# balisujohn/tortoise.cpp

Hardware: AMD Instinct MI355X
Metric: audio-seconds/sec end-to-end (AR+diffusion+vocoder), 16 cands x 80 steps (higher is better)
Workload: dtype f16 MFMA inputs / f32 accumulate (diffusion, vocoder convs); f32 weights, f16 KV (AR)

## Files before the change

tortoise.cpp_amd/csrc/diffusion.hip:

```cpp
#include "common.h"
#include "gemm_f16.h"
#include <algorithm>
#include <chrono>
#include <cmath>

namespace tts {

static constexpr int C = 1024, NHEAD = 16, XTC = 128 ;
static constexpr int LAT_MAX_ROWS = 2048;
static constexpr int HOIST_MAX_ROWS = 16384;

__device__ __forceinline__ float silu_dev(float x, int lut) {
  if (lut == 1) {
    float xr = __half2float(__float2half_rn(x));
    return __half2float(__float2half_rn(xr / (1.0f + expf(-xr))));
  }
  if (lut == 2) return x / (1.0f + expf(-x));
  return x * __builtin_amdgcn_rcpf(1.0f + __builtin_amdgcn_exp2f(x * -1.44269504088896f));
}

__global__ __launch_bounds__(256) void gn_stats_kernel(const float *__restrict__ x, const int *__restrict__ seq_start,
                                                       const int *__restrict__ seq_len, float eps, float2 *__restrict__ stats) {
  __shared__ float sh[8];
  const int grp = blockIdx.x, s = blockIdx.y, T = seq_len[s];
// ... 1213 lines not shown
    if (g.mode == GEMM_OUT_QKV) fam = "diff_gemm_qkv";
    else if (gemm_is_conv3(g) && g.N == C && g.kseg == C) fam = g.resid ? "diff_gemm_k3r" : "diff_gemm_k3";
    else if (g.nseg == 1 && g.N == C && g.kseg == C && g.mode == GEMM_OUT_F32) fam = g.resid ? "diff_gemm_k1r" : "diff_gemm_k1";
    else if (g.custom_w && g.N == C && g.kseg == C && g.mode == GEMM_OUT_F32_SCALED && g.resid) fam = "diff_gemm_k1r";
    else fam = "diff_gemm_misc";
  }
  ProfScope ps(ctx, fam, 2.0 * mv * (n_valid ? n_valid : g.N) * (k_valid ? k_valid : g.nseg * g.kseg));
  TTS_HIP(ctx, launch_gemm_f16(g, ctx->stream));
  if (ctx->fp16_check) {
    if (gemm_mode_qkv(g.mode)) {
      CHECK(fp16_check(ctx, g.outH, (size_t)g.M * g.ldh));
      CHECK(fp16_check(ctx, g.outVt, (size_t)(g.N / 3) * g.ldvt));
    } else if (g.mode == GEMM_OUT_F16) CHECK(fp16_check(ctx, g.outH, (size_t)g.M * g.ldh));
  }
  return TTS_OK;
}

static int gemm_wreg_class(const tts_ctx *ctx, int bit) { return (ctx->gemm_wreg & bit) ? 1 : 0; }
static const __half *gemm_wreg_image(const tts_ctx *ctx, int bit, const Layout &lay, int N, const __half *w, const __half *wf) {
  return gemm_wreg_class(ctx, bit) && gemm_auto_th(lay.rows, N) == 8 ? wf : w;
}

static GemmArgs gemm_base(const Layout &lay, const __half *A, int lda, int nseg, int kseg, const __half *W, int N,
                          const float *bias) {
  GemmArgs g{};
  for (int i = 0; i < 3; i++) { g.A[i] = A; g.row_off[i] = 0; }
  if (nseg == 3) { g.row_off[0] = -1; g.row_off[1] = 0; g.row_off[2] = 1; }
  g.nseg = nseg; g.kseg = kseg; g.lda = lda; g.W = W; g.M = lay.rows; g.N = N; g.bias = bias;
  g.row_seq = lay.d_row_seq.as<int>();
  return g;
}

static int gn_stats(tts_ctx *ctx, const Layout &lay, Work &wk, const float *x) {
  ProfScope ps(ctx, "diff_gn_stats");
  gn_stats_kernel<<<dim3(32, lay.ns), 256, 0, ctx->stream>>>(x, lay.d_start.as<int>(), lay.d_len.as<int>(), ctx->gn_eps,
                                                             wk.stats.as<float2>());
  TTS_HIP(ctx, hipGetLastError());
  return TTS_OK;
}
template <int NT, int NJ, class LOAD, class TOUCH>
__device__ __forceinline__ void gn_reg_body(LOAD load, TOUCH touch, int s, int c, int T, int r0, const int *__restrict__ seq_start, int rows_total, int ns, float eps,
                                            const float *__restrict__ g, const float *__restrict__ b, const float *__restrict__ ss, int do_silu, int lut,
                                            __half *__restrict__ y, const int *__restrict__ seq_step, int ss_step_stride) {
  constexpr int NW = NT / 64, SWEEP = NT / 8;
  __shared__ float sh[2][NW];
  const int t0 = threadIdx.x >> 3;
  float4 v[NJ];
#pragma unroll
  for (int j = 0; j < NJ; j++) {
    const int t = t0 + j * SWEEP;
    v[j] = load(min(t, T - 1));
  }
  touch();
  const float4 gg = *(const float4 *)(g + c), bb = *(const float4 *)(b + c);
  float sc4[4] = {1.f, 1.f, 1.f, 1.f}, sh4[4] = {0.f, 0.f, 0.f, 0.f};
  if (ss) {
    if (seq_step) ss += (size_t)seq_step[s] * ss_step_stride;
#pragma unroll
    for (int i = 0; i < 4; i++) { sc4[i] = ss[c + i] + 1.0f; sh4[i] = ss[C + c + i]; }
  }
  float sum = 0.f;
#pragma unroll
  for (int j = 0; j < NJ; j++)
    if (t0 + j * SWEEP < T) sum += (v[j].x + v[j].y) + (v[j].z + v[j].w);
#pragma unroll
  for (int o = 32; o > 0; o >>= 1) sum += __shfl_xor(sum, o);
  if ((threadIdx.x & 63) == 0) sh[0][threadIdx.x >> 6] = sum;
  __syncthreads();
  float tot = 0.f;
#pragma unroll
  for (int w = 0; w < NW; w++) tot += sh[0][w];
  const float n = (float)T * 32.f, mean = tot / n;
  float sq = 0.f;
#pragma unroll
  for (int j = 0; j < NJ; j++) {
    v[j].x -= mean; v[j].y -= mean; v[j].z -= mean; v[j].w -= mean;
    if (t0 + j * SWEEP < T) sq += (v[j].x * v[j].x + v[j].y * v[j].y) + (v[j].z * v[j].z + v[j].w * v[j].w);
  }
#pragma unroll
  for (int o = 32; o > 0; o >>= 1) sq += __shfl_xor(sq, o);
  if ((threadIdx.x & 63) == 0) sh[1][threadIdx.x >> 6] = sq;
  __syncthreads();
  float tsq = 0.f;
#pragma unroll
  for (int w = 0; w < NW; w++) tsq += sh[1][w];
  const float rstd = 1.0f / sqrtf(tsq / n + eps);
  const float ge[4] = {gg.x, gg.y, gg.z, gg.w}, be[4] = {bb.x, bb.y, bb.z, bb.w};
  auto apply = [&](auto mode) {
    constexpr int MODE = decltype(mode)::value;
#pragma unroll
    for (int j = 0; j < NJ; j++) {
      const int t = min(t0 + j * SWEEP, T - 1);
      float e[4] = {v[j].x, v[j].y, v[j].z, v[j].w};
#pragma unroll
      for (int i = 0; i < 4; i++) {
        float u = e[i] * rstd;
        u = u * ge[i];
        u = u + be[i];
        u = u * sc4[i];
        u = u + sh4[i];
        if (MODE) u = silu_dev(u, MODE - 1);
        e[i] = u;
      }
      const __half2 p0 = __floats2half2_rn(e[0], e[1]), p1 = __floats2half2_rn(e[2], e[3]);
      uint2 o;
      o.x = *(const unsigned *)&p0;
      o.y = *(const unsigned *)&p1;
      *(uint2 *)(y + (size_t)(r0 + t) * C + c) = o;
    }
  };
  if (!do_silu) apply(std::integral_constant<int, 0>{});
  else if (lut == 0) apply(std::integral_constant<int, 1>{});
  else if (lut == 1) apply(std::integral_constant<int, 2>{});
  else apply(std::integral_constant<int, 3>{});
  const int gend = (s + 1 < ns) ? seq_start[s + 1] : rows_total;
  for (int r = r0 + T + t0; r < gend; r += SWEEP) *(uint2 *)(y + (size_t)r * C + c) = make_uint2(0u, 0u);
  if (s == 0)
    for (int r = t0; r < r0; r += SWEEP) *(uint2 *)(y + (size_t)r * C + c) = make_uint2(0u, 0u);
}
template <int NT, int NJ>
__global__ __launch_bounds__(NT) void gn_reg_kernel(const float *__restrict__ x, const int *__restrict__ seq_start,
                                                    const int *__restrict__ seq_len, int rows_total, int ns, float eps,
                                                    const float *__restrict__ g, const float *__restrict__ b,
                                                    const float *__restrict__ ss, int do_silu, int lut, __half *__restrict__ y,
                                                    const char *__restrict__ pf0, int pf0_lines, const char *__restrict__ pf1, int pf1_lines,
                                                    const int *__restrict__ seq_step, int ss_step_stride) {
  constexpr int NW = NT / 64;
  __shared__ unsigned pf_sink[NW][64];
  const int bid = blockIdx.y * 32 + blockIdx.x, nbk = ns * 32, item = (bid & 7) * (nbk >> 3) + (bid >> 3);
  const int s = item >> 5, grp = item & 31;
  const int T = seq_len[s], r0 = seq_start[s];
  const int q = threadIdx.x & 7, c = grp * 32 + q * 4;
  const float *base = x + (size_t)r0 * C + c;
  auto touch = [&]() {
    const int gi = (blockIdx.y * 32 + blockIdx.x) * NT + threadIdx.x, tt = 32 * ns * NT;
    unsigned *sink = &pf_sink[__builtin_amdgcn_readfirstlane(threadIdx.x >> 6)][0];
    for (int l = gi; l < pf0_lines; l += tt) __builtin_amdgcn_global_load_lds((gptr_t)(pf0 + (size_t)l * 128), (lptr_t)sink, 4, 0, 0);
    for (int l = gi; l < pf1_lines; l += tt) __builtin_amdgcn_global_load_lds((gptr_t)(pf1 + (size_t)l * 128), (lptr_t)sink, 4, 0, 0);
  };
  gn_reg_body<NT, NJ>([&](int t) { return *(const float4 *)(base + (size_t)t * C); }, touch, s, c, T, r0, seq_start, rows_total, ns, eps, g, b, ss, do_silu, lut, y, seq_step,
                      ss_step_stride);
  if (pf0_lines | pf1_lines) asm volatile("s_waitcnt vmcnt(0)" ::: "memory");
}
struct GnPanelTail {
  __device__ __forceinline__ void operator()(const GemmGnPanelArgs &a, int s, int T, int r0, int c0, const char *panel) const {
    const int q = threadIdx.x & 7;
    gn_reg_body<512, 14>([&](int t) { return *(const float4 *)(panel + gnp_panel_f4(t, q)); }, []() {}, s, c0 + q * 4, T, r0, a.seq_start, a.rows_total, a.ns, a.eps, a.gn_g,
                         a.gn_b, a.ss, a.do_silu, a.lut, a.y, a.seq_step, a.ss_step_stride);
  }
};

static inline hipError_t launch_gemm_gn_panel(const GemmGnPanelArgs &a, hipStream_t s) {
  static bool raised = false;
  if (!raised) { (void)hipFuncSetAttribute((const void *)gemm_f16_gn_panel_kernel<GnPanelTail>, hipFuncAttributeMaxDynamicSharedMemorySize, GEMM_GN_PANEL_LDS); raised = true; }
  gemm_f16_gn_panel_kernel<GnPanelTail><<<gemm_gn_panel_grid(a.ns, a.N), 512, GEMM_GN_PANEL_LDS, s>>>(a, GnPanelTail{});
  return hipGetLastError();
}

static int gn_fused(tts_ctx *ctx, const Layout &lay, const float *x, const float *g, const float *b, const float *ss, int do_silu,
                    __half *y, const void *wa = nullptr, size_t wa_bytes = 0, const void *wb = nullptr, size_t wb_bytes = 0) {
  ProfScope ps(ctx, "diff_gn_fused");
  if (lay.rows > 4096) { wa_bytes = 0; wb_bytes = 0; }
  const int silu_mode = ctx->ggml_lut ? 1 : ctx->attn_f32 ? 2 : 0;
  auto launch = [&](const int *d_start, int s0, int ns, int row0, int rows, int tmax) {
    const float *xp = x + (size_t)row0 * C;
    __half *yp = y + (size_t)row0 * C;
    const int *d_len = lay.d_len.as<int>() + s0, *step = lay.seq_step_ptr() ? lay.seq_step_ptr() + s0 : nullptr;
#define GN_ARGS xp, d_start, d_len, rows, ns, ctx->gn_eps, g, b, ss, do_silu, silu_mode, yp, \
                (const char *)wa, (int)(wa_bytes >> 7), (const char *)wb, (int)(wb_bytes >> 7), step, lay.ss_step_stride
    if (tmax <= 14 * 64) gn_reg_kernel<512, 14><<<dim3(32, ns), 512, 0, ctx->stream>>>(GN_ARGS);
    else if (tmax <= 18 * 128) gn_reg_kernel<1024, 18><<<dim3(32, ns), 1024, 0, ctx->stream>>>(GN_ARGS);
    else gn_fused_kernel<0><<<dim3(32, ns), 256, 0, ctx->stream>>>(xp, d_start, d_len, rows, ns, ctx->gn_eps, g, b, ss,
                                                                  do_silu, silu_mode, yp, step, lay.ss_step_stride);
#undef GN_ARGS
  };
  if (lay.gn_parts.empty()) launch(lay.d_start.as<int>(), 0, lay.ns, 0, lay.rows, lay.max_len());
  else for (const Layout::GnPart &p : lay.gn_parts) launch(lay.d_start_rel.as<int>() + p.s0, p.s0, p.ns, p.row0, p.rows, p.tmax);
  TTS_HIP(ctx, hipGetLastError());
  return TTS_OK;
}

__global__ __launch_bounds__(256) void gn_apply_kernel(const float *__restrict__ x, const int *__restrict__ chunk_seq, const int *__restrict__ seq_start,
                                                       const int *__restrict__ seq_len, const long long *__restrict__ st, int stripe_ll, float eps, const float *__restrict__ g,
                                                       const float *__restrict__ b, const float *__restrict__ ss, int do_silu, int lut, __half *__restrict__ y,
                                                       const char *__restrict__ pf0, int pf0_lines, const char *__restrict__ pf1, int pf1_lines,
                                                       const int *__restrict__ seq_step, int ss_step_stride) {
  __shared__ float2 mr[32];
  __shared__ unsigned pf_sink[4][64];
  const int r0 = blockIdx.x * 4, s = chunk_seq[blockIdx.x >> 1], c = threadIdx.x * 4;
  float4 v[4];
#pragma unroll
  for (int r = 0; r < 4; r++) v[r] = *(const float4 *)(x + (size_t)(r0 + r) * C + c);
  {
    const int gi = blockIdx.x * 256 + threadIdx.x, tt = gridDim.x * 256;
    unsigned *sink = &pf_sink[__builtin_amdgcn_readfirstlane(threadIdx.x >> 6)][0];
    for (int l = gi; l < pf0_lines; l += tt) __builtin_amdgcn_global_load_lds((gptr_t)(pf0 + (size_t)l * 128), (lptr_t)sink, 4, 0, 0);
    for (int l = gi; l < pf1_lines; l += tt) __builtin_amdgcn_global_load_lds((gptr_t)(pf1 + (size_t)l * 128), (lptr_t)sink, 4, 0, 0);
  }
  int nvalid = 0;
  if (s >= 0) {
    nvalid = min(max(seq_start[s] + seq_len[s] - r0, 0), 4);
    if (threadIdx.x < 32) {
      long long a[4] = {0, 0, 0, 0};
      longlong2 u[FX_STRIPES][2];
#pragma unroll
      for (int k = 0; k < FX_STRIPES; k++) {
        const long long *sp = st + (size_t)k * stripe_ll + (size_t)(s * 32 + threadIdx.x) * 4;
        u[k][0] = *(const longlong2 *)sp; u[k][1] = *(const longlong2 *)(sp + 2);
      }
#pragma unroll
      for (int k = 0; k < FX_STRIPES; k++) { a[0] += u[k][0].x; a[1] += u[k][0].y; a[2] += u[k][1].x; a[3] += u[k][1].y; }
      const double n = (double)seq_len[s] * 32.0;
      const double mean = fx_value(a[0], a[1]) / n;
      const double var = fmax(fx_value(a[2], a[3]) / n - mean * mean, 0.0);
      mr[threadIdx.x] = make_float2((float)mean, (float)(1.0 / sqrt(var + (double)eps)));
    }
  }
  __syncthreads();
  const float2 m = mr[c >> 5];
  const float4 gg = *(const float4 *)(g + c), bb = *(const float4 *)(b + c);
  float sc4[4] = {1.f, 1.f, 1.f, 1.f}, sh4[4] = {0.f, 0.f, 0.f, 0.f};
  if (ss) {
    if (seq_step && s >= 0) ss += (size_t)seq_step[s] * ss_step_stride;
#pragma unroll
    for (int i = 0; i < 4; i++) { sc4[i] = ss[c + i] + 1.0f; sh4[i] = ss[C + c + i]; }
  }
  const float ge[4] = {gg.x, gg.y, gg.z, gg.w}, be[4] = {bb.x, bb.y, bb.z, bb.w};
  auto apply = [&](auto mode) {
    constexpr int MODE = decltype(mode)::value;
#pragma unroll
    for (int r = 0; r < 4; r++) {
      float e[4] = {v[r].x, v[r].y, v[r].z, v[r].w};
#pragma unroll
      for (int i = 0; i < 4; i++) {
        float u = (e[i] - m.x) * m.y;
        u = u * ge[i];
        u = u + be[i];
        u = u * sc4[i];
        u = u + sh4[i];
        if (MODE) u = silu_dev(u, MODE - 1);
        e[i] = r < nvalid ? u : 0.f;
      }
      const __half2 p0 = __floats2half2_rn(e[0], e[1]), p1 = __floats2half2_rn(e[2], e[3]);
      uint2 o;
      o.x = *(const unsigned *)&p0;
      o.y = *(const unsigned *)&p1;
      *(uint2 *)(y + (size_t)(r0 + r) * C + c) = o;
    }
  };
  if (!do_silu) apply(std::integral_constant<int, 0>{});
  else if (lut == 0) apply(std::integral_constant<int, 1>{});
  else if (lut == 1) apply(std::integral_constant<int, 2>{});
  else apply(std::integral_constant<int, 3>{});
  if (pf0_lines | pf1_lines) asm volatile("s_waitcnt vmcnt(0)" ::: "memory");
}

static int gn(tts_ctx *ctx, const DiffState *st, const Layout &lay, const float *x, const long long *st_x, const float *g, const float *b, const float *ss, int do_silu,
              __half *y, const void *wa = nullptr, size_t wa_bytes = 0, const void *wb = nullptr, size_t wb_bytes = 0) {
  if (!st_x) {
    CHECK(gn_fused(ctx, lay, x, g, b, ss, do_silu, y, wa, wa_bytes, wb, wb_bytes));
    return fp16_check(ctx, y, (size_t)lay.rows * C);
  }
  {
    ProfScope ps(ctx, "diff_gn_apply");
    const int silu_mode = ctx->ggml_lut ? 1 : ctx->attn_f32 ? 2 : 0;
    gn_apply_kernel<<<lay.rows / 4, 256, 0, ctx->stream>>>(x, lay.d_chunk_seq.as<int>(), lay.d_start.as<int>(), lay.d_len.as<int>(), st_x, (int)st->gn_stripe_ll, ctx->gn_eps, g, b,
                                                            ss, do_silu, silu_mode, y, (const char *)wa, (int)(wa_bytes >> 7), (const char *)wb, (int)(wb_bytes >> 7),
                                                            lay.seq_step_ptr(), lay.ss_step_stride);
    TTS_HIP(ctx, hipGetLastError());
  }
  return fp16_check(ctx, y, (size_t)lay.rows * C);
}

static int res_in_layers(tts_ctx *ctx, const DiffState *st, const Layout &lay, Work &wk, const float *x, const ResDev &w, float *H,
                         const long long *st_x = nullptr, long long *st_h_out = nullptr) {
  CHECK(gn(ctx, st, lay, x, st_x, w.in_g, w.in_b, nullptr, 1, wk.A16(), gemm_wreg_image(ctx, 1, lay, C, w.in_w, w.in_wf), (size_t)C * C * 2));
  DBG_SUM("res.in gn", wk.A16(), (size_t)lay.rows * C * 2);
  GemmArgs g = gemm_base(lay, wk.A16(), C, 1, C, w.in_w, C, w.in_bias);
  g.mode = st_h_out ? GEMM_OUT_F32_STATS : GEMM_OUT_F32; g.outF = H; g.ldo = C; g.resid = nullptr;
  g.Wf = w.in_wf; g.wreg = gemm_wreg_class(ctx, 1);
  g.st_out = st_h_out; g.st_stripe_ll = (int)st->gn_stripe_ll; g.chunk_seq = lay.d_chunk_seq.as<int>();
  CHECK(gemm(ctx, "diff_gemm", g, lay));
  DBG_SUM("res.in conv", H, (size_t)lay.rows * C * 4);
  return TTS_OK;
}

static int attention_block(tts_ctx *ctx, DiffState *st, const Layout &lay, Work &wk, float *X, const AttnDev &w, bool force_ref = false) {
  const bool f32 = ctx->attn_f32 != 0 || force_ref;
  const bool pw16 = !f32 && ctx->attn_proj_f16;
  const bool lat = st->lat && wk.st_x != nullptr;
  CHECK(gn(ctx, st, lay, X, lat ? wk.st_x : nullptr, w.norm_g, w.norm_b, nullptr, 0, wk.A16(), gemm_wreg_image(ctx, 2, lay, 3 * C, w.qkv_w, w.qkv_wf), (size_t)3 * C * C * 2, pw16 ? w.proj_w : w.proj_w_split,
           (size_t)C * C * (pw16 ? 2 : 4)));
  long long *st_out = lat ? st->new_stats_slot() : nullptr;
  wk.st_x = st_out;
  DBG_SUM("attn gn", wk.A16(), (size_t)lay.rows * C * 2);
  GemmArgs g = gemm_base(lay, wk.A16(), C, 1, C, w.qkv_w, 3 * C, w.qkv_b);
  g.mode = f32 ? GEMM_OUT_QKV_SPLIT : GEMM_OUT_QKV;
  g.Wf = w.qkv_wf; g.wreg = gemm_wreg_class(ctx, 2);
  g.outH = wk.qk16.as<__half>(); g.ldh = 2048; g.outVt = wk.vt16.as<__half>(); g.ldvt = wk.rows + 128;
  g.outH2 = wk.qk16_lo.as<__half>(); g.outVt2 = wk.vt16_lo.as<__half>();
  CHECK(gemm(ctx, "diff_gemm", g, lay));
  if (f32 && (ctx->attn_f32_drop & 1)) TTS_HIP(ctx, hipMemsetAsync(wk.qk16_lo.p, 0, (size_t)(wk.rows + 128) * 2048 * 2, ctx->stream));
  if (f32 && (ctx->attn_f32_drop & 2)) TTS_HIP(ctx, hipMemsetAsync(wk.vt16_lo.p, 0, (size_t)C * (wk.rows + 128) * 2, ctx->stream));
  DBG_SUM("attn qk", wk.qk16.p, (size_t)lay.rows * 2048 * 2);
  DBG_SUM("attn vt", wk.vt16.p, (size_t)C * (wk.rows + 128) * 2);
  {
    double aw = 0;
    for (int l : lay.len) aw += 4.0 * l * (double)l * 64 * NHEAD;
// ... 920 lines not shown
```

tortoise.cpp_amd/csrc/gemm_f16.h:

```cpp
#pragma once
#include <hip/hip_fp16.h>
#include <hip/hip_runtime.h>
#include <algorithm>
#include <cmath>
#include <cstdlib>
#include <type_traits>

namespace tts {

typedef _Float16 half8 __attribute__((ext_vector_type(8)));
typedef float floatx4 __attribute__((ext_vector_type(4)));

enum { GEMM_OUT_F32 = 0, GEMM_OUT_F16 = 1, GEMM_OUT_QKV = 2, GEMM_OUT_QKV_SPLIT = 3, GEMM_OUT_F32_SCALED = 4, GEMM_OUT_F32_STATS = 5, GEMM_OUT_F32_SCALED_STATS = 6 };
constexpr bool gemm_mode_qkv(int mode) { return mode == GEMM_OUT_QKV || mode == GEMM_OUT_QKV_SPLIT; }
constexpr bool gemm_mode_f32(int mode) { return mode == GEMM_OUT_F32 || mode == GEMM_OUT_F32_SCALED || mode == GEMM_OUT_F32_STATS || mode == GEMM_OUT_F32_SCALED_STATS; }
constexpr bool gemm_mode_scaled(int mode) { return mode == GEMM_OUT_F32_SCALED || mode == GEMM_OUT_F32_SCALED_STATS; }
constexpr bool gemm_mode_stats(int mode) { return mode == GEMM_OUT_F32_STATS || mode == GEMM_OUT_F32_SCALED_STATS; }

struct GemmArgs {
  const __half *A[3];
  int row_off[3];
  int nseg, kseg;
  int lda;
  const __half *W;
// ... 493 lines not shown
      return;
    }
  }
  const int col0 = c0 + fq * 4;
  float4 b4[2];
  int sq[MI];
#pragma unroll
  for (int j = 0; j < 2; j++) b4[j] = *(const float4 *)(bp + col0 + j * 16);
#pragma unroll
  for (int i = 0; i < MI; i++) sq[i] = sp[m0 + min(i, nblk - 1) * 16 + fr];
#pragma unroll
  for (int j = 0; j < 2; j++) b4[j] = hb ? b4[j] : make_float4(0.f, 0.f, 0.f, 0.f);
#pragma unroll
  for (int i = 0; i < MI; i++) sq[i] = hs ? sq[i] : 0;
  auto finish = [&](int i, int j) {
    float4 v = make_float4(acc[i][j][0] + b4[j].x, acc[i][j][1] + b4[j].y, acc[i][j][2] + b4[j].z, acc[i][j][3] + b4[j].w);
    if (sq[i] < 0) v = make_float4(0.f, 0.f, 0.f, 0.f);
    return v;
  };
  if (MODE == GEMM_OUT_F32) {
#pragma unroll
    for (int i = 0; i < MI; i++) {
      if (i < nblk) {
        float *op = g.outF + (size_t)(m0 + i * 16 + fr) * g.ldo + col0;
#pragma unroll
        for (int j = 0; j < 2; j++) *(float4 *)(op + j * 16) = finish(i, j);
      }
    }
  } else {
    const int h = c0 / 192, w0 = c0 - h * 192;
#pragma unroll
    for (int i = 0; i < MI; i++) {
      if (i < nblk) {
        __half *op = g.outH + (size_t)(m0 + i * 16 + fr) * g.ldh + h * 128 + w0 + fq * 4;
#pragma unroll
        for (int j = 0; j < 2; j++) {
          const float4 v = finish(i, j);
          *(uint2 *)(op + j * 16) = pack_half4(v.x, v.y, v.z, v.w);
          if (MODE == GEMM_OUT_QKV_SPLIT)
            *(uint2 *)(g.outH2 + (op - g.outH) + j * 16) = pack_half4(split_lo(v.x), split_lo(v.y), split_lo(v.z), split_lo(v.w));
        }
      }
    }
  }
}

template <int MODE, int MI, int D, bool NAT>
__device__ __forceinline__ void gemm_wreg_body(const GemmArgs &g, int m0, int n0, int nblk, int lane, int wave) {
  extern __shared__ __attribute__((aligned(16))) char smem_dyn[];
  char *smem = smem_dyn;
  constexpr int S = D + 1;
  constexpr int NPA = MI / 2;
  constexpr int PER = NPA + 4;
  static_assert(D == 1 || D == 2, "prefetch distance");
  const int T = g.kseg >> 6, KS = g.kseg >> 5;
  const int fr = lane & 15, fq = lane >> 4;
  unsigned aoff[NPA];
#pragma unroll
  for (int i = 0; i < NPA; i++) aoff[i] = (unsigned)(gemm_dma_off(wave + 4 * i, lane, 0, nblk * 16 - 1, g.lda) * 2);
  const char *aseg = (const char *)(g.A[0] + (ptrdiff_t)(g.row_off[0] + m0) * g.lda);
  const __half *wp0 = g.Wf + (size_t)((n0 >> 4) + wave * 2) * KS * 512, *wp1 = wp0 + (size_t)KS * 512;
  const unsigned wlane = lane * 16;
  const bool resid_first = MODE == GEMM_OUT_F32 && g.resid != nullptr;
  floatx4 acc[MI][2];
  gemm_acc_start<MODE, MI, 2>(g, acc, resid_first, n0 + wave * 32, fq, [&](int i) { return m0 + min(i, nblk - 1) * 16 + fr; });
  half8 w[S][2][2];
  auto issue = [&](int t, auto set_c) {
    constexpr int U = decltype(set_c)::value;
    const char *ab = aseg + (t << 7);
#pragma unroll
    for (int i = 0; i < NPA; i++) __builtin_amdgcn_global_load_lds((gptr_t)(ab + aoff[i]), (lptr_t)(smem + U * 16384 + (wave + 4 * i) * 1024), 16, 0, 0);
    const __half *q0 = wp0 + (size_t)t * 1024, *q1 = wp1 + (size_t)t * 1024;
    wreg_load<0>(w[U][0][0], q0, wlane);
    wreg_load<0>(w[U][0][1], q1, wlane);
    wreg_load<1024>(w[U][1][0], q0, wlane);
    wreg_load<1024>(w[U][1][1], q1, wlane);
  };
  auto kloop = [&]() {
    auto step = [&](int t, auto u_c) {
      constexpr int U = decltype(u_c)::value;
      if (D == 2 && t + 1 < T) wreg_wait<PER>(w[U][0][0], w[U][0][1], w[U][1][0], w[U][1][1]);
      else wreg_wait<0>(w[U][0][0], w[U][0][1], w[U][1][0], w[U][1][1]);
      asm volatile("s_waitcnt lgkmcnt(0)" ::: "memory");
      __builtin_amdgcn_s_barrier();
      if (t + D < T) issue(t + D, std::integral_constant<int, (U + D) % S>{});
      const char *sa = smem + U * 16384;
      constexpr int AHEAD = 2;
      half8 af[AHEAD + 1];
      auto frag = [&](int x) { return *(const half8 *)(sa + lds_off((x % MI) * 16 + fr, (x / MI) * 4 + fq)); };
#pragma unroll
      for (int x = 0; x < AHEAD; x++) af[x] = frag(x);
#pragma unroll
      for (int x = 0; x < 2 * MI; x++) {
        if (x + AHEAD < 2 * MI) af[(x + AHEAD) % (AHEAD + 1)] = frag(x + AHEAD);
        const int ks = x / MI, i = x % MI;
        const half8 a = af[x % (AHEAD + 1)];
#pragma unroll
        for (int j = 0; j < 2; j++) {
          if (NAT) acc[i][j] = __builtin_amdgcn_mfma_f32_16x16x32_f16(a, w[U][ks][j], acc[i][j], 0, 0, 0);
          else acc[i][j] = __builtin_amdgcn_mfma_f32_16x16x32_f16(w[U][ks][j], a, acc[i][j], 0, 0, 0);
        }
      }
      __builtin_amdgcn_sched_group_barrier(0x100, AHEAD, 0);
#pragma unroll
      for (int x = 0; x < 2 * MI; x++) {
        if (x + AHEAD < 2 * MI) __builtin_amdgcn_sched_group_barrier(0x100, 1, 0);
        __builtin_amdgcn_sched_group_barrier(0x008, 2, 0);
      }
    };
    for (int t0 = 0; t0 < T; t0 += S) {
      step(t0, std::integral_constant<int, 0>{});
      if (t0 + 1 < T) step(t0 + 1, std::integral_constant<int, 1>{});
      if (S == 3 && t0 + 2 < T) step(t0 + 2, std::integral_constant<int, S - 1>{});
    }
  };
  issue(0, std::integral_constant<int, 0>{});
  if (D == 2) issue(1, std::integral_constant<int, 1>{});
#pragma unroll
  for (int i = 0; i < MI; i++)
#pragma unroll
    for (int j = 0; j < 2; j++) asm volatile("" : "+v"(acc[i][j]));
  kloop();
  gemm_epilogue_wreg<MODE, MI, NAT>(g, acc, m0, n0, nblk, wave, fr, fq);
}

static constexpr int GEMM_WREG_D = 1, GEMM_WREG_LDS = (GEMM_WREG_D + 1) * 16384;
template <int MODE, int D = GEMM_WREG_D>
static __global__ __launch_bounds__(256, 4) void gemm_f16_wreg_kernel(GemmArgs g) {
  const int tid = threadIdx.x, lane = tid & 63, wave = __builtin_amdgcn_readfirstlane(tid >> 6);
  int m0, n0, nblk;
  if (!gemm_vh_tile(g, m0, n0, nblk)) return;
  if (gemm_mode_qkv(MODE) && ((n0 + wave * 32) % 192) >= 128) {
    if (nblk > 4) gemm_wreg_body<MODE, 8, D, true>(g, m0, n0, nblk, lane, wave);
    else gemm_wreg_body<MODE, 4, D, true>(g, m0, n0, nblk, lane, wave);
  } else {
    if (nblk > 4) gemm_wreg_body<MODE, 8, D, false>(g, m0, n0, nblk, lane, wave);
    else gemm_wreg_body<MODE, 4, D, false>(g, m0, n0, nblk, lane, wave);
  }
}
static inline bool gemm_takes_wreg(const GemmArgs &g, int th, int ku) {
  return g.wreg > 0 && g.Wf && g.nseg == 1 && !g.custom_w && th == 8 && ku == 1 && (g.kseg >> 6) >= 2 &&
         (g.mode == GEMM_OUT_F32 || g.mode == GEMM_OUT_QKV || g.mode == GEMM_OUT_QKV_SPLIT);
}

struct GemmGnPanelArgs {
  const __half *A; int lda;
  const __half *Wf;
  int N, K;
  const float *bias;
  const int *seq_start, *seq_len; int ns, rows_total;
  float eps; const float *gn_g, *gn_b, *ss; int do_silu, lut; __half *y; const int *seq_step; int ss_step_stride;
};
static constexpr int GEMM_GN_PANEL_ROWS = 896, GEMM_GN_PANEL_LDS = GEMM_GN_PANEL_ROWS * 128;
__device__ __forceinline__ int gnp_panel_f4(int t, int q) { return t * 128 + ((q ^ (t & 7)) << 4); }
template <int OFF> __device__ __forceinline__ void gnp_lds_read(half8 &d, unsigned addr) {
  asm volatile("ds_read_b128 %0, %1 offset:%2" : "=v"(d) : "v"(addr), "i"(OFF));
}
static inline int gemm_auto_th(int M, int N);
static inline bool gemm_gn_panel_takes(int option, bool stats, bool debug_sums, bool has_wf, int max_len, int rows, int N, int K) {
  return option != 0 && !stats && !debug_sums && has_wf && max_len >= 1 && max_len <= GEMM_GN_PANEL_ROWS && gemm_auto_th(rows, N) == 8 && (N % 64) == 0 && K >= 64 && (K % 64) == 0;
}
static inline int gemm_gn_panel_grid(int ns, int N) { return 8 * ((ns * (N >> 6) + 7) / 8); }

template <class TAIL>
static __global__ __launch_bounds__(512) void gemm_f16_gn_panel_kernel(GemmGnPanelArgs a, TAIL tail) {
  extern __shared__ __attribute__((aligned(16))) char smem_dyn[];
  char *smem = smem_dyn;
  const int tid = threadIdx.x, lane = tid & 63, wave = __builtin_amdgcn_readfirstlane(tid >> 6);
  const int np = a.N >> 6, nitems = a.ns * np, xcd = blockIdx.x & 7, idx = blockIdx.x >> 3;
  const int i0 = (int)((long long)nitems * xcd >> 3), i1 = (int)((long long)nitems * (xcd + 1) >> 3);
  if (idx >= i1 - i0) return;
  const int item = i0 + idx, s = item / np, n0 = (item - s * np) << 6;
  const int T = a.seq_len[s], r0 = a.seq_start[s];
  const int KT = a.K >> 6, fr = lane & 15, fq = lane >> 4;
  const int rb = wave * 8 + (lane >> 3), lda2 = a.lda * 2;
  const unsigned coloff = (unsigned)(((lane & 7) ^ lds_swz(lane >> 3)) << 4);
  const char *aseg = (const char *)(a.A + (size_t)r0 * a.lda);
  const size_t wstride = (size_t)(a.K >> 5) * 512;
  const __half *wp0 = a.Wf + (size_t)(n0 >> 4) * wstride, *wp1 = wp0 + wstride, *wp2 = wp1 + wstride, *wp3 = wp2 + wstride;
  const unsigned wlane = lane * 16;
  const unsigned lds0 = (unsigned)(size_t)(lptr_t)smem + wave * 7 * 2048;
  const unsigned fb0 = lds0 + lds_off(fr, fq), fb1 = lds0 + lds_off(fr, 4 + fq);
  floatx4 acc[7][4];
#pragma unroll
  for (int i = 0; i < 7; i++)
#pragma unroll
    for (int j = 0; j < 4; j++) acc[i][j] = (floatx4){0.f, 0.f, 0.f, 0.f};
  half8 w[2][4];
  auto dma = [&](int t) {
    const char *ab = aseg + (t << 7);
    int rbv = rb;
    asm volatile("" : "+v"(rbv));
#pragma unroll
    for (int i = 0; i < 14; i++) {
      const unsigned off = (unsigned)(min(rbv + 64 * i, T - 1) * lda2) + coloff;
      __builtin_amdgcn_global_load_lds((gptr_t)(ab + off), (lptr_t)(smem + (wave + 8 * i) * 1024), 16, 0, 0);
    }
  };
  auto wload = [&](int t, auto ks_c) {
    constexpr int KS = decltype(ks_c)::value;
    const size_t o = (size_t)t * 1024;
    wreg_load<KS * 1024>(w[KS][0], wp0 + o, wlane);
    wreg_load<KS * 1024>(w[KS][1], wp1 + o, wlane);
    wreg_load<KS * 1024>(w[KS][2], wp2 + o, wlane);
    wreg_load<KS * 1024>(w[KS][3], wp3 + o, wlane);
  };
  auto pin_acc = [&]() {
#pragma unroll
    for (int j = 0; j < 4; j++)
      asm volatile("" : "+v"(acc[0][j]), "+v"(acc[1][j]), "+v"(acc[2][j]), "+v"(acc[3][j]), "+v"(acc[4][j]), "+v"(acc[5][j]), "+v"(acc[6][j]));
  };
  auto step = [&](int t, auto last_c) {
    constexpr bool LAST = decltype(last_c)::value;
    wreg_wait<4>(w[0][0], w[0][1], w[0][2], w[0][3]);
    __builtin_amdgcn_s_barrier();
    asm volatile("" ::: "memory");
    half8 af[2][7];
    gnp_lds_read<0 * 2048>(af[0][0], fb0);
    gnp_lds_read<1 * 2048>(af[0][1], fb0);
    gnp_lds_read<2 * 2048>(af[0][2], fb0);
    gnp_lds_read<3 * 2048>(af[0][3], fb0);
    gnp_lds_read<4 * 2048>(af[0][4], fb0);
    gnp_lds_read<5 * 2048>(af[0][5], fb0);
    gnp_lds_read<6 * 2048>(af[0][6], fb0);
    gnp_lds_read<0 * 2048>(af[1][0], fb1);
    gnp_lds_read<1 * 2048>(af[1][1], fb1);
    gnp_lds_read<2 * 2048>(af[1][2], fb1);
    gnp_lds_read<3 * 2048>(af[1][3], fb1);
    gnp_lds_read<4 * 2048>(af[1][4], fb1);
    gnp_lds_read<5 * 2048>(af[1][5], fb1);
    gnp_lds_read<6 * 2048>(af[1][6], fb1);
    asm volatile("s_waitcnt lgkmcnt(0)"
                 : "+v"(af[0][0]), "+v"(af[0][1]), "+v"(af[0][2]), "+v"(af[0][3]), "+v"(af[0][4]), "+v"(af[0][5]), "+v"(af[0][6]), "+v"(af[1][0]), "+v"(af[1][1]),
                   "+v"(af[1][2]), "+v"(af[1][3]), "+v"(af[1][4]), "+v"(af[1][5]), "+v"(af[1][6])
                 :
                 : "memory");
    __builtin_amdgcn_s_barrier();
    asm volatile("" ::: "memory");
    if (!LAST) dma(t + 1);
#pragma unroll
    for (int i = 0; i < 7; i++)
#pragma unroll
      for (int j = 0; j < 4; j++) acc[i][j] = __builtin_amdgcn_mfma_f32_16x16x32_f16(w[0][j], af[0][i], acc[i][j], 0, 0, 0);
    if (!LAST) {
      pin_acc();
      wload(t + 1, std::integral_constant<int, 0>{});
    }
    wreg_wait<LAST ? 0 : 18>(w[1][0], w[1][1], w[1][2], w[1][3]);
#pragma unroll
    for (int i = 0; i < 7; i++)
#pragma unroll
      for (int j = 0; j < 4; j++) acc[i][j] = __builtin_amdgcn_mfma_f32_16x16x32_f16(w[1][j], af[1][i], acc[i][j], 0, 0, 0);
    if (!LAST) {
      pin_acc();
      wload(t + 1, std::integral_constant<int, 1>{});
    }
  };
  dma(0);
  wload(0, std::integral_constant<int, 0>{});
  wload(0, std::integral_constant<int, 1>{});
  for (int t = 0; t + 1 < KT; t++) step(t, std::false_type{});
  step(KT - 1, std::true_type{});
  const bool hb = a.bias != nullptr;
  const float *bp = hb ? a.bias : (const float *)a.Wf;
  float4 b4[4];
#pragma unroll
  for (int j = 0; j < 4; j++) b4[j] = *(const float4 *)(bp + n0 + j * 16 + fq * 4);
#pragma unroll
  for (int j = 0; j < 4; j++) b4[j] = hb ? b4[j] : make_float4(0.f, 0.f, 0.f, 0.f);
#pragma unroll
  for (int gi = 0; gi < 2; gi++) {
#pragma unroll
    for (int i = 0; i < 7; i++) {
      const int row = (wave * 7 + i) * 16 + fr;
#pragma unroll
      for (int jj = 0; jj < 2; jj++) {
        const int j = gi * 2 + jj;
        *(float4 *)(smem + gnp_panel_f4(row, jj * 4 + fq)) = make_float4(acc[i][j][0] + b4[j].x, acc[i][j][1] + b4[j].y, acc[i][j][2] + b4[j].z, acc[i][j][3] + b4[j].w);
      }
    }
    __syncthreads();
    tail(a, s, T, r0, n0 + gi * 32, smem);
  }
}

static constexpr int CONV3_VH_LDS = (128 + 8) * 128 + 2 * 16384;
template <int MODE, int MI>
__device__ __forceinline__ void gemm_conv3_vh_body(const GemmArgs &g, int m0, int n0, int nblk, int lane, int wave) {
  extern __shared__ __attribute__((aligned(16))) char smem_dyn[];
  char *smem = smem_dyn;
  constexpr int MA = MI > 0 ? MI : 1;
  const int wm = wave >> 1, wn = wave & 1;
  const int my_pa = (2 * nblk + 1 - wave + 3) >> 2;
  const int nchunks = g.kseg >> 6, ldw = 3 * g.kseg, nph = 3 * nchunks;
  const int prow = lane >> 3, pslot = lane & 7;
  const int fr = lane & 15, fq = lane >> 4;
  floatx4 acc[MA][4];
#pragma unroll
  for (int i = 0; i < MI; i++)
#pragma unroll
    for (int j = 0; j < 4; j++) acc[i][j] = (floatx4){0.f, 0.f, 0.f, 0.f};
  char *sa = smem, *sb = smem + (128 + 8) * 128;
  const __half *abase = g.A[0] + (ptrdiff_t)(m0 - 1) * g.lda;
  const __half *wbase = g.W + (size_t)n0 * ldw;
  int aoff[5], boff[4];
#pragma unroll
  for (int i = 0; i < 5; i++) {
    const int row = (wave + 4 * i) * 8 + prow;
    aoff[i] = min(row, g.M - m0 + 1) * g.lda + (pslot ^ lds_swz(row)) * 8;
  }
#pragma unroll
  for (int i = 0; i < 4; i++) {
    const int row = (wave * 4 + i) * 8 + prow;
    boff[i] = row * ldw + (pslot ^ lds_swz(row)) * 8;
  }
  auto stageA = [&](int kc) {
    const __half *src = abase + (min(kc, nchunks - 1) << 6);
#pragma unroll
    for (int i = 0; i < 5; i++)
      if (i < my_pa) __builtin_amdgcn_global_load_lds((gptr_t)(src + aoff[i]), (lptr_t)(sa + (wave + 4 * i) * 1024), 16, 0, 0);
  };
  auto stageB = [&](int p) {
    p = min(p, nph - 1);
    const int kc = p / 3, tap = p - kc * 3;
    const __half *src = wbase + tap * g.kseg + (kc << 6);
    char *dst = sb + (p & 1) * 16384;
#pragma unroll
    for (int i = 0; i < 4; i++) __builtin_amdgcn_global_load_lds((gptr_t)(src + boff[i]), (lptr_t)(dst + (wave * 4 + i) * 1024), 16, 0, 0);
  };
  auto phase = [&](int kc, int p, auto tap_c) {
    constexpr int TAP = decltype(tap_c)::value;
    stageB(p + 1);
    asm volatile("s_waitcnt vmcnt(4)" ::: "memory");
    __builtin_amdgcn_s_barrier();
    const char *sbp = sb + (p & 1) * 16384;
#pragma unroll
    for (int ks = 0; ks < 2; ks++) {
      half8 af[MA], bf[4];
#pragma unroll
      for (int i = 0; i < MI; i++) af[i] = *(const half8 *)(sa + lds_off(vh_blk(wm, i) * 16 + fr + TAP, ks * 4 + fq));
      if (MI > 0) {
#pragma unroll
        for (int i = 0; i < 4; i++) bf[i] = *(const half8 *)(sbp + lds_off(wn * 64 + i * 16 + fr, ks * 4 + fq));
      }
#pragma unroll
      for (int i = 0; i < MI; i++)
#pragma unroll
        for (int j = 0; j < 4; j++) acc[i][j] = __builtin_amdgcn_mfma_f32_16x16x32_f16(bf[j], af[i], acc[i][j], 0, 0, 0);
    }
    asm volatile("s_waitcnt lgkmcnt(0)" ::: "memory");
    __builtin_amdgcn_s_barrier();
    if (TAP == 2) stageA(kc + 1);
  };
  stageA(0);
  stageB(0);
  for (int kc = 0; kc < nchunks; kc++) {
    const int p = 3 * kc;
    phase(kc, p, std::integral_constant<int, 0>{});
    phase(kc, p + 1, std::integral_constant<int, 1>{});
    phase(kc, p + 2, std::integral_constant<int, 2>{});
  }
  asm volatile("s_waitcnt vmcnt(0)" ::: "memory");
  if ((MODE == GEMM_OUT_F32 || MODE == GEMM_OUT_F32_STATS) && g.resid) gemm_epilogue_vh<MODE, MI, EPI_RESID_LOAD>(g, acc, m0, n0, wm, wn, fr, fq);
  else gemm_epilogue_vh<MODE, MI, EPI_NO_RESID>(g, acc, m0, n0, wm, wn, fr, fq);
}

template <int MODE>
static __global__ __launch_bounds__(256, 3) void gemm_f16_conv3_vh_kernel(GemmArgs g) {
  const int tid = threadIdx.x, lane = tid & 63, wave = __builtin_amdgcn_readfirstlane(tid >> 6);
  int m0, n0, nblk;
  if (!gemm_vh_tile(g, m0, n0, nblk)) return;
  gemm_for_my_mi(nblk, wave, [&](auto mi) { gemm_conv3_vh_body<MODE, decltype(mi)::value>(g, m0, n0, nblk, lane, wave); });
}

static inline bool gemm_is_conv3(const GemmArgs &g) {
  return g.nseg == 3 && !g.custom_w && g.A[0] == g.A[1] && g.A[1] == g.A[2] && g.row_off[0] == -1 && g.row_off[1] == 0 && g.row_off[2] == 1 &&
         !gemm_mode_qkv(g.mode) && !gemm_mode_scaled(g.mode);
}

static inline size_t gemm_wfrag3_index(int n, int tap, int k, int N, int K) {
  return (size_t)tap * N * K + gemm_wfrag_index(n, k, K);
}
static constexpr int CONV3_WREG_SLOT = (128 + 8) * 128, CONV3_WREG_LDS = 2 * CONV3_WREG_SLOT;

template <int MI, bool RESID>
__device__ __forceinline__ void gemm_epilogue_conv3_wreg(const GemmArgs &g, floatx4 (&acc)[MI][2], int m0, int n0, int nblk, int wave, int fr, int fq) {
  const int col0 = n0 + wave * 32 + fq * 4;
  const bool hb = g.bias != nullptr, hs = g.row_seq != nullptr;
  const float *bp = hb ? g.bias : (const float *)g.W;
  const int *sp = hs ? g.row_seq : (const int *)g.A[0];
  float4 b4[2], rr[2][2];
  int sq[MI];
  auto load_pair = [&](int p) {
#pragma unroll
    for (int q = 0; q < 2; q++) {
      const float *rp = g.resid + (size_t)(m0 + min(2 * p + q, nblk - 1) * 16 + fr) * g.ldo + col0;
#pragma unroll
      for (int j = 0; j < 2; j++) rr[q][j] = *(const float4 *)(rp + j * 16);
    }
  };
  if (RESID) load_pair(0);
#pragma unroll
  for (int j = 0; j < 2; j++) b4[j] = *(const float4 *)(bp + col0 + j * 16);
#pragma unroll
  for (int i = 0; i < MI; i++) sq[i] = sp[m0 + min(i, nblk - 1) * 16 + fr];
#pragma unroll
  for (int j = 0; j < 2; j++) b4[j] = hb ? b4[j] : make_float4(0.f, 0.f, 0.f, 0.f);
#pragma unroll
  for (int i = 0; i < MI; i++) sq[i] = hs ? sq[i] : 0;
#pragma unroll
  for (int p = 0; p < MI / 2; p++) {
    float4 v[2][2];
#pragma unroll
// ... 233 lines not shown
```

Before: 142.0.

## Stage GEMM-GN panel weights through a double-buffered LDS ring via async DMA

New measurement: 143.8, median of 6. 1.3% higher.

```diff
diff --git a/tortoise.cpp_amd/csrc/diffusion.hip b/tortoise.cpp_amd/csrc/diffusion.hip
--- a/tortoise.cpp_amd/csrc/diffusion.hip
+++ b/tortoise.cpp_amd/csrc/diffusion.hip
@@ -1389,8 +1389,8 @@
 
 static inline hipError_t launch_gemm_gn_panel(const GemmGnPanelArgs &a, hipStream_t s) {
   static bool raised = false;
-  if (!raised) { (void)hipFuncSetAttribute((const void *)gemm_f16_gn_panel_kernel<GnPanelTail>, hipFuncAttributeMaxDynamicSharedMemorySize, GEMM_GN_PANEL_LDS); raised = true; }
-  gemm_f16_gn_panel_kernel<GnPanelTail><<<gemm_gn_panel_grid(a.ns, a.N), 512, GEMM_GN_PANEL_LDS, s>>>(a, GnPanelTail{});
+  if (!raised) { (void)hipFuncSetAttribute((const void *)gemm_f16_gn_panel_kernel<GnPanelTail>, hipFuncAttributeMaxDynamicSharedMemorySize, GEMM_GN_PANEL_LDS_LAUNCH); raised = true; }
+  gemm_f16_gn_panel_kernel<GnPanelTail><<<gemm_gn_panel_grid(a.ns, a.N), 512, GEMM_GN_PANEL_LDS_LAUNCH, s>>>(a, GnPanelTail{});
   return hipGetLastError();
 }
 
diff --git a/tortoise.cpp_amd/csrc/gemm_f16.h b/tortoise.cpp_amd/csrc/gemm_f16.h
--- a/tortoise.cpp_amd/csrc/gemm_f16.h
+++ b/tortoise.cpp_amd/csrc/gemm_f16.h
@@ -669,6 +669,7 @@
   float eps; const float *gn_g, *gn_b, *ss; int do_silu, lut; __half *y; const int *seq_step; int ss_step_stride;
 };
 static constexpr int GEMM_GN_PANEL_ROWS = 896, GEMM_GN_PANEL_LDS = GEMM_GN_PANEL_ROWS * 128;
+static constexpr int GEMM_GN_PANEL_WRING = 2 * 8192, GEMM_GN_PANEL_LDS_LAUNCH = GEMM_GN_PANEL_LDS + GEMM_GN_PANEL_WRING;
 __device__ __forceinline__ int gnp_panel_f4(int t, int q) { return t * 128 + ((q ^ (t & 7)) << 4); }
 template <int OFF> __device__ __forceinline__ void gnp_lds_read(half8 &d, unsigned addr) {
   asm volatile("ds_read_b128 %0, %1 offset:%2" : "=v"(d) : "v"(addr), "i"(OFF));
@@ -690,12 +691,13 @@
   const int item = i0 + idx, s = item / np, n0 = (item - s * np) << 6;
   const int T = a.seq_len[s], r0 = a.seq_start[s];
   const int KT = a.K >> 6, fr = lane & 15, fq = lane >> 4;
-  const int rb = wave * 8 + (lane >> 3), lda2 = a.lda * 2;
+  const int rb = wave * 112 + (lane >> 3), lda2 = a.lda * 2;
   const unsigned coloff = (unsigned)(((lane & 7) ^ lds_swz(lane >> 3)) << 4);
   const char *aseg = (const char *)(a.A + (size_t)r0 * a.lda);
   const size_t wstride = (size_t)(a.K >> 5) * 512;
-  const __half *wp0 = a.Wf + (size_t)(n0 >> 4) * wstride, *wp1 = wp0 + wstride, *wp2 = wp1 + wstride, *wp3 = wp2 + wstride;
-  const unsigned wlane = lane * 16;
+  const __half *wsrc = a.Wf + (size_t)((n0 >> 4) + (wave & 3)) * wstride + (wave >> 2) * 512 + lane * 8;
+  char *wring = smem + GEMM_GN_PANEL_LDS;
+  const unsigned wfb = (unsigned)(size_t)(lptr_t)wring + lane * 16;
   const unsigned lds0 = (unsigned)(size_t)(lptr_t)smem + wave * 7 * 2048;
   const unsigned fb0 = lds0 + lds_off(fr, fq), fb1 = lds0 + lds_off(fr, 4 + fq);
   floatx4 acc[7][4];
@@ -703,36 +705,21 @@
   for (int i = 0; i < 7; i++)
 #pragma unroll
     for (int j = 0; j < 4; j++) acc[i][j] = (floatx4){0.f, 0.f, 0.f, 0.f};
-  half8 w[2][4];
   auto dma = [&](int t) {
     const char *ab = aseg + (t << 7);
     int rbv = rb;
     asm volatile("" : "+v"(rbv));
 #pragma unroll
     for (int i = 0; i < 14; i++) {
-      const unsigned off = (unsigned)(min(rbv + 64 * i, T - 1) * lda2) + coloff;
-      __builtin_amdgcn_global_load_lds((gptr_t)(ab + off), (lptr_t)(smem + (wave + 8 * i) * 1024), 16, 0, 0);
-    }
-  };
-  auto wload = [&](int t, auto ks_c) {
-    constexpr int KS = decltype(ks_c)::value;
-    const size_t o = (size_t)t * 1024;
-    wreg_load<KS * 1024>(w[KS][0], wp0 + o, wlane);
-    wreg_load<KS * 1024>(w[KS][1], wp1 + o, wlane);
-    wreg_load<KS * 1024>(w[KS][2], wp2 + o, wlane);
-    wreg_load<KS * 1024>(w[KS][3], wp3 + o, wlane);
-  };
-  auto pin_acc = [&]() {
-#pragma unroll
-    for (int j = 0; j < 4; j++)
-      asm volatile("" : "+v"(acc[0][j]), "+v"(acc[1][j]), "+v"(acc[2][j]), "+v"(acc[3][j]), "+v"(acc[4][j]), "+v"(acc[5][j]), "+v"(acc[6][j]));
-  };
+      const unsigned off = (unsigned)(min(rbv + 8 * i, T - 1) * lda2) + coloff;
+      __builtin_amdgcn_global_load_lds((gptr_t)(ab + off), (lptr_t)(smem + (wave * 14 + i) * 1024), 16, 0, 0);
+    }
+  };
+  auto wdma = [&](int t) { __builtin_amdgcn_global_load_lds((gptr_t)(wsrc + (size_t)t * 1024), (lptr_t)(wring + ((t & 1) << 13) + wave * 1024), 16, 0, 0); };
   auto step = [&](int t, auto last_c) {
     constexpr bool LAST = decltype(last_c)::value;
-    wreg_wait<4>(w[0][0], w[0][1], w[0][2], w[0][3]);
-    __builtin_amdgcn_s_barrier();
-    asm volatile("" ::: "memory");
-    half8 af[2][7];
+    asm volatile("s_waitcnt vmcnt(1)" ::: "memory");
+    half8 af[2][7], w[2][4];
     gnp_lds_read<0 * 2048>(af[0][0], fb0);
     gnp_lds_read<1 * 2048>(af[0][1], fb0);
     gnp_lds_read<2 * 2048>(af[0][2], fb0);
@@ -752,30 +739,32 @@
                    "+v"(af[1][2]), "+v"(af[1][3]), "+v"(af[1][4]), "+v"(af[1][5]), "+v"(af[1][6])
                  :
                  : "memory");
+    if (!LAST) dma(t + 1);
+    if (LAST) asm volatile("s_waitcnt vmcnt(0)" ::: "memory");
+    else asm volatile("s_waitcnt vmcnt(14)" ::: "memory");
     __builtin_amdgcn_s_barrier();
     asm volatile("" ::: "memory");
-    if (!LAST) dma(t + 1);
-#pragma unroll
-    for (int i = 0; i < 7; i++)
-#pragma unroll
-      for (int j = 0; j < 4; j++) acc[i][j] = __builtin_amdgcn_mfma_f32_16x16x32_f16(w[0][j], af[0][i], acc[i][j], 0, 0, 0);
-    if (!LAST) {
-      pin_acc();
-      wload(t + 1, std::integral_constant<int, 0>{});
-    }
-    wreg_wait<LAST ? 0 : 18>(w[1][0], w[1][1], w[1][2], w[1][3]);
-#pragma unroll
-    for (int i = 0; i < 7; i++)
-#pragma unroll
-      for (int j = 0; j < 4; j++) acc[i][j] = __builtin_amdgcn_mfma_f32_16x16x32_f16(w[1][j], af[1][i], acc[i][j], 0, 0, 0);
-    if (!LAST) {
-      pin_acc();
-      wload(t + 1, std::integral_constant<int, 1>{});
-    }
+    if (!LAST) wdma(t + 1);
+    const unsigned wf = wfb + ((t & 1) << 13);
+    gnp_lds_read<0 * 1024>(w[0][0], wf);
+    gnp_lds_read<1 * 1024>(w[0][1], wf);
+    gnp_lds_read<2 * 1024>(w[0][2], wf);
+    gnp_lds_read<3 * 1024>(w[0][3], wf);
+    gnp_lds_read<4 * 1024>(w[1][0], wf);
+    gnp_lds_read<5 * 1024>(w[1][1], wf);
+    gnp_lds_read<6 * 1024>(w[1][2], wf);
+    gnp_lds_read<7 * 1024>(w[1][3], wf);
+    asm volatile("s_waitcnt lgkmcnt(0)" : "+v"(w[0][0]), "+v"(w[0][1]), "+v"(w[0][2]), "+v"(w[0][3]), "+v"(w[1][0]), "+v"(w[1][1]), "+v"(w[1][2]), "+v"(w[1][3]) : : "memory");
+    __builtin_amdgcn_sched_barrier(0);
+#pragma unroll
+    for (int ks = 0; ks < 2; ks++)
+#pragma unroll
+      for (int i = 0; i < 7; i++)
+#pragma unroll
+        for (int j = 0; j < 4; j++) acc[i][j] = __builtin_amdgcn_mfma_f32_16x16x32_f16(w[ks][j], af[ks][i], acc[i][j], 0, 0, 0);
   };
   dma(0);
-  wload(0, std::integral_constant<int, 0>{});
-  wload(0, std::integral_constant<int, 1>{});
+  wdma(0);
   for (int t = 0; t + 1 < KT; t++) step(t, std::false_type{});
   step(KT - 1, std::true_type{});
   const bool hb = a.bias != nullptr;
```
